# albanie/mcnCrossModalEmotions

Hardware: AMD Instinct MI355X
Metric: distillation-step samples/sec (face+audio pair) (higher is better)
Workload: dtype f32; 1 GPU; BASELINE config 4 shard: frozen resnet50 teacher fwd + VGGVox student fwd/bwd/SGD; per_gpu_batch=32, global_batch=32, face=224x224x3, teacher_batch=32, spectrogram=512x300x1, parallelism=dp1, weights=random-init (seeded), parameter_server=rccl-capi, streams=teacher one batch ahead on its own stream + wgrad side stream

## Files before the change

### mcncrossmodalemotions_amd/csrc/context.cpp

```cpp
#include <cstdlib>
#include <map>
#include <string>
#include <vector>

#include "xm_common.h"

namespace xm {
bool path_on(Path p) {
  static const char *const kEnv[kPathCount] = {"XM_NO_HYBRID",      "XM_NO_HALO",        "XM_NO_SKINNY",     "XM_NO_SKINNY4",
                                               "XM_NO_STEM",        "XM_NO_STEM_WGRAD",  "XM_NO_DMA",        "XM_NO_FUSED_STATS",
                                               "XM_DGRAD_MERGE",    "XM_NO_FAST_TRANSPOSE", "XM_NO_POOL_LDS", "XM_NO_POOL_PATCH",
                                               "XM_NO_POOL_POOLED", "XM_NO_W8", "XM_NO_WGRAD_PATCH", "XM_NO_WGRAD_PATCH_S2", "XM_NO_DGRAD_S2", "XM_NO_STEM3"};
  static bool on[kPathCount];
  static bool read = false;
  if (!read) {
    for (int i = 0; i < kPathCount; ++i) on[i] = getenv(kEnv[i]) == nullptr;
    read = true;
  }
  return on[p];
}

long long env_int(const char *name, long long dflt) {
  const char *e = getenv(name);
  return (e && *e) ? atoll(e) : dflt;
}
double env_double(const char *name, double dflt) {
  const char *e = getenv(name);
  return (e && *e) ? atof(e) : dflt;
}

static char g_err[512] = "";
char *err_buf() { return g_err; }

int fail(int code, const char *fmt, ...) {
  va_list ap;
  va_start(ap, fmt);
  vsnprintf(g_err, sizeof g_err, fmt, ap);
  va_end(ap);
  return code;
}

struct WsBuf {
  void *ptr = nullptr;
  size_t cap = 0;
};
static std::map<hipStream_t, WsBuf> g_ws;
static unsigned long long g_ws_generation = 0;

int ws_get(size_t bytes, void **ptr, hipStream_t stream) {
  WsBuf &w = g_ws[stream];
  if (bytes > w.cap) {
    size_t want = bytes + bytes / 4 + (1u << 20);
    static const bool verbose = getenv("XM_WS_VERBOSE") != nullptr;
    if (verbose) fprintf(stderr, "[xm ws] stream %p grow %zu -> %zu\n", (void *)stream, w.cap, want);
    ++g_ws_generation;
    if (w.ptr) {
      hipError_t e = hipDeviceSynchronize();
      if (e != hipSuccess) return fail(XM_EHIP, "hipDeviceSynchronize -> %s", hipGetErrorString(e));
      (void)hipFree(w.ptr);
      w.ptr = nullptr;
      w.cap = 0;
    }
    hipError_t e = hipMalloc(&w.ptr, want);
    if (e != hipSuccess) {
      w.ptr = nullptr;
      return fail(XM_ENOMEM, "workspace hipMalloc(%zu) -> %s", want, hipGetErrorString(e));
    }
    w.cap = want;
  }
  *ptr = w.ptr;
  return XM_OK;
}

static std::map<std::string, void *> g_tables;

const void *cached_device_table(const void *host, size_t bytes) {
  std::string key((const char *)host, bytes);
  auto it = g_tables.find(key);
  if (it != g_tables.end()) return it->second;
  void *d = nullptr;
  static const bool verbose = getenv("XM_WS_VERBOSE") != nullptr;
  if (verbose) fprintf(stderr, "[xm ws] new device table %zu bytes (#%zu)\n", bytes, g_tables.size());
  if (hipMalloc(&d, bytes) != hipSuccess) return nullptr;
  if (hipMemcpy(d, host, bytes, hipMemcpyHostToDevice) != hipSuccess) {
    (void)hipFree(d);
    return nullptr;
  }
  g_tables.emplace(std::move(key), d);
  return d;
}

}

extern "C" {

int xm_version(void) { return 106; }
const char *xm_last_error(void) { return xm::err_buf(); }

int xm_workspace_reserve(size_t bytes) {
  void *p;
  return xm::ws_get(bytes, &p, nullptr);
}
int xm_workspace_reserve_stream(size_t bytes, void *stream) {
  void *p;
  return xm::ws_get(bytes, &p, (hipStream_t)stream);
}
unsigned long long xm_workspace_generation(void) { return xm::g_ws_generation; }

int xm_device_alloc(void **ptr, size_t bytes) {
  if (!ptr) return xm::fail(XM_EINVAL, "device_alloc: NULL output");
  *ptr = nullptr;
  if (bytes == 0) return XM_OK;
  hipError_t e = hipMalloc(ptr, bytes);
  if (e != hipSuccess) return xm::fail(XM_ENOMEM, "hipMalloc(%zu) -> %s", bytes, hipGetErrorString(e));
  return XM_OK;
}
int xm_device_free(void *ptr) {
  if (!ptr) return XM_OK;
  hipError_t e = hipFree(ptr);
  if (e != hipSuccess) return xm::fail(XM_EHIP, "hipFree -> %s", hipGetErrorString(e));
  return XM_OK;
}
int xm_device_upload(void *dst_device, const void *src_host, size_t bytes) {
  if (bytes == 0) return XM_OK;
// ... 28 lines not shown
```

### mcncrossmodalemotions_amd/csrc/conv.hip

```cpp
#include <dlfcn.h>

#include <algorithm>
#include <climits>
#include <cstdlib>
#include <map>
#include <string>
#include <vector>

#include "conv_kernels.h"
#include "stem_pool_kernels.h"

namespace xm {


__global__ void pad_filter_kernel(const float *__restrict__ f, float *__restrict__ o, int M, int R,
                                  int Rp) {
  size_t i = blockIdx.x * (size_t)blockDim.x + threadIdx.x;
  if (i >= (size_t)M * Rp) return;
  int r = (int)(i % Rp);
  size_t m = i / Rp;
  o[i] = r < R ? f[m * R + r] : 0.f;
}

struct PrepDiv {
// ... 337 lines not shown
  ProfScope(int key, double flops, hipStream_t s, double bytes = 0) : on(g_prof_on), st(s) {
    if (!on) return;
    r.key = key;
    r.flops = flops;
    r.bytes = bytes;
    r.start = prof_event();
    r.stop = prof_event();
    (void)hipEventRecord(r.start, st);
  }
  ~ProfScope() {
    if (!on) return;
    (void)hipEventRecord(r.stop, st);
    g_prof.push_back(r);
  }
};


static const int kCfgOcc[kNumBaseCfg] = {2, 2, 2, 3, 4, 3, 4, 2};

static int hybrid_plan(const ConvGemmArgs &a, int ci, int *full_out) {
  const bool off = !path_on(kPathHybrid);
  *full_out = 0;
  if (off || is_dma_cfg(ci) || g_force_splits > 0) return 1;
  if (a.statPart && (!a.vecStore || a.relu || a.resid)) return 1;
  const int tiles = a.nbm * a.nbn, slots = 256 * kCfgOcc[ci];
  if (tiles <= slots || a.nkt < 16) return 1;
  int full = tiles / slots * slots;
  full -= full % a.nbm;
  const int rem = tiles - full;
  if (rem <= 0 || rem * 5 > slots * 4) return 1;
  const int S = std::min(std::min(slots / rem, a.nkt / 8), 16);
  if (S < 2) return 1;
  *full_out = full;
  return S;
}

static size_t gemm_slab_floats(const ConvGemmArgs &a, int ci, int *splits_out) {
  const Cfg &c = kCfgs[ci];
  int nbm = (a.M + c.bm() - 1) / c.bm(), nbn = (a.NP + c.bn() - 1) / c.bn();
  int splits = pick_splits(nbm * nbn, a.Rp / kBK);
  *splits_out = splits;
  size_t need = splits > 1 ? (size_t)splits * a.M * ((a.NP + 3) & ~3) : 0;
  if (splits == 1 && !is_dma_cfg(ci)) {
    ConvGemmArgs t = a;
    t.nbm = nbm, t.nbn = nbn, t.nkt = a.Rp / kBK;
    t.statPart = nullptr;
    int full;
    const int S = hybrid_plan(t, ci, &full);
    if (S > 1) need = std::max(need, (size_t)S * a.M * ((size_t)(nbm * nbn - full) / nbm * c.bn() + 4));
  }
  return need;
}

static int launch_gemm(ConvGemmArgs &a, int mode, int ci, int splits, float *slab, hipStream_t st) {
  if (is_dma_cfg(ci) && !a.dmaOk) ci = base_cfg(ci);
  if (ci == kCfgW8 && !path_on(kPathW8)) ci = 0;
  const Cfg &c = kCfgs[ci];
  a.nbm = (a.M + c.bm() - 1) / c.bm();
  a.nbn = (a.NP + c.bn() - 1) / c.bn();
  a.nkt = a.Rp / kBK;
  a.tilesPerSplit = (a.nkt + splits - 1) / splits;
  splits = (a.nkt + a.tilesPerSplit - 1) / a.tilesPerSplit;
  a.NPs = (a.NP + 3) & ~3;
  a.slab = splits > 1 ? slab : nullptr;
  a.dbgCycles = g_dbg_cycles;
  a.hyS = 1, a.hyFull = 0, a.hyTps = 0, a.hyP0 = 0;
  dim3 grid(a.nbm * a.nbn, splits);
  int hyS = 1;
  if (splits == 1 && slab) {
    int full;
    hyS = hybrid_plan(a, ci, &full);
    if (hyS > 1) {
      a.hyFull = full;
      a.hyTps = (a.nkt + hyS - 1) / hyS;
      hyS = (a.nkt + a.hyTps - 1) / a.hyTps;
      a.hyS = hyS;
      a.hyP0 = full / a.nbm * c.bn();
      a.NPs = (a.NP - a.hyP0 + 3) & ~3;
      a.slab = slab;
      grid = dim3(full + (a.nbm * a.nbn - full) * hyS, 1);
    }
  }
  {
    const double abytes = (double)a.xBytes + 4.0 * a.M * a.Rtrue + 4.0 * a.M * (double)a.NP * (a.resid ? 2 : 1);
    ProfScope ps(0 * 100 + ci * 2 + mode, a.algoFlops > 0 ? a.algoFlops : 2.0 * a.M * (double)a.NP * a.Rtrue, st,
                 abytes);
    if (is_dma_cfg(ci)) {
      static const int per_cu_tab[] = XM_DMA_PERCU;
      const int slots = std::max(8, 256 * per_cu_tab[ci - kNumBaseCfg] / std::max(1, splits));
      const int ntl = a.nbm * a.nbn;
      const int g = ntl <= slots ? ntl : slots - slots % 8;
      launch_gemm_dma(ci, a, dim3(std::max(1, g), splits), st);
    } else if (mode)
      launch_gemm_cfg<1>(ci, a, grid, st);
    else
      launch_gemm_cfg<0>(ci, a, grid, st);
  }
  XM_LAUNCH_CHECK();
  if (splits > 1 || hyS > 1) {
    const int z = splits > 1 ? splits : hyS;
    const int np = a.NP - a.hyP0;
    const bool vec = a.vecStore && (np & 3) == 0 && (a.hyP0 & 3) == 0 && (a.NPs & 3) == 0 && ((uintptr_t)a.slab & 15) == 0;
    const size_t n = (size_t)a.M * (vec ? np / 4 : np);
    if (hyS > 1 && a.statPart) {
      const int cols = np / 4, chunks = (cols + 255) / 256, statBase = a.hyFull / a.nbm;
      if (!vec) return fail(XM_EINVAL, "vl_nnconv: hybrid schedule with statistics needs vector stores");
      hipLaunchKernelGGL(conv_splitk_epilogue_stats_kernel, dim3(chunks, a.M), dim3(256), 0, st, a, z, cols, statBase);
      a.statNcg = statBase + chunks;
    } else if (vec)
      hipLaunchKernelGGL(conv_splitk_epilogue_kernel<true>, dim3((unsigned)((n + 255) / 256)), dim3(256), 0, st,
                         a, z, make_fastdiv((uint32_t)(np / 4)));
    else
      hipLaunchKernelGGL(conv_splitk_epilogue_kernel<false>, dim3((unsigned)((n + 255) / 256)), dim3(256), 0, st,
                         a, z, make_fastdiv((uint32_t)np));
    XM_LAUNCH_CHECK();
  }
  return XM_OK;
}

static void launch_gemm_multi_cfg(int ci, const ConvGemmMulti &m, dim3 grid, hipStream_t st) {
  dim3 block(cfg_threads(ci));
  switch (ci) {
    case 7: hipLaunchKernelGGL((conv_gemm_multi_kernel<1, 2, 4, 2>), grid, block, 0, st, m); break;
    case 0: hipLaunchKernelGGL((conv_gemm_multi_kernel<2, 2, 2, 2>), grid, block, 0, st, m); break;
    case 1: hipLaunchKernelGGL((conv_gemm_multi_kernel<2, 2, 1, 4>), grid, block, 0, st, m); break;
    case 2: hipLaunchKernelGGL((conv_gemm_multi_kernel<3, 1, 1, 4>), grid, block, 0, st, m); break;
    case 3: hipLaunchKernelGGL((conv_gemm_multi_kernel<1, 2, 2, 2>), grid, block, 0, st, m); break;
    case 4: hipLaunchKernelGGL((conv_gemm_multi_kernel<1, 1, 2, 2>), grid, block, 0, st, m); break;
    case 5: hipLaunchKernelGGL((conv_gemm_multi_kernel<1, 1, 4, 1>), grid, block, 0, st, m); break;
    default: hipLaunchKernelGGL((conv_gemm_multi_kernel<1, 1, 1, 4>), grid, block, 0, st, m); break;
  }
}

static int launch_gemm_multi(const std::vector<ConvGemmArgs> &args, int ci, hipStream_t st) {
  ci = base_cfg(ci);
  if (ci == kCfgW8 && !path_on(kPathW8)) ci = 0;
  const Cfg &c = kCfgs[ci];
  ConvGemmMulti m{};
  int maxTiles = 0;
  double flops = 0, abytes = args.empty() ? 0.0 : (double)args[0].xBytes;
  for (size_t i = 0; i < args.size(); ++i) {
    ConvGemmArgs a = args[i];
    a.nbm = (a.M + c.bm() - 1) / c.bm();
    a.nbn = (a.NP + c.bn() - 1) / c.bn();
    a.nkt = a.Rp / kBK;
    a.tilesPerSplit = a.nkt;
    a.NPs = (a.NP + 3) & ~3;
    a.slab = nullptr;
    maxTiles = std::max(maxTiles, a.nbm * a.nbn);
    flops += a.algoFlops > 0 ? a.algoFlops : 2.0 * a.M * (double)a.NP * a.Rtrue;
    abytes += 4.0 * a.M * a.Rtrue + 4.0 * a.M * (double)a.NP * (a.resid ? 2 : 1);
    m.c[i] = a;
  }
  {
    ProfScope ps(2 * 100 + ci * 2, flops, st, abytes);
    launch_gemm_multi_cfg(ci, m, dim3(maxTiles, 1, (unsigned)args.size()), st);
// ... 35 lines not shown
    const long long p1 = std::min<long long>(p0 + BN - 1, a.NP - 1);
    const long long c0 = (p0 / pij) * a.hpWP + (p0 % pij) / a.PI, c1 = (p1 / pij) * a.hpWP + (p1 % pij) / a.PI;
    worst = std::max(worst, (int)(c1 - c0) + a.nV);
  }
  return worst * a.hpHP;
}
static int halo_setup_padded(ConvGemmArgs &a, int nSamples) {
  int need = halo_setup(a, nSamples);
  if (need <= 512 || a.vecStore || a.slab) return need;
  const int piv = (a.PI + 31) / 32 * 32;
  if (piv == a.PI || (piv - a.PI) * 25 > piv || (long long)piv * a.PJ * nSamples >= (1LL << 31)) return need;
  ConvGemmArgs b = a;
  b.piReal = a.PI;
  b.PI = piv;
  b.NP = piv * a.PJ * nSamples;
  b.divPI = make_fastdiv((uint32_t)piv);
  b.divPIJ = make_fastdiv((uint32_t)(piv * a.PJ));
  const int need2 = halo_setup(b, nSamples);
  if (need2 > 0 && need2 <= 512) {
    a = b;
    return need2;
  }
  return need;
}

static bool halo_var_ok(const ConvGemmArgs &a, int need, int v) {
  if (need <= 0 || need > kHaloVars[v].ps) return false;
  if (v == 2 && need <= 512) return false;
  if (kHaloVars[v].bm == 96 && (a.M % 96 != 0)) return false;
  return true;
}

static int halo_splits(const ConvGemmArgs &a, int v) {
  const int bm = kHaloVars[v].bm;
  const int tiles = ((a.M + bm - 1) / bm) * ((a.NP + 127) / 128), nst = a.Rtrue / (kHaloCB * a.nU * a.nV);
  if (tiles >= 384 || nst < 8) return 1;
  return std::max(1, std::min(std::min(512 / tiles, nst / 4), 16));
}
static size_t halo_slab_floats(const ConvGemmArgs &a) {
  int sp = 1;
  for (int v = 0; v < 3; ++v) sp = std::max(sp, halo_splits(a, v));
  return sp > 1 ? (size_t)sp * a.M * ((a.NP + 3) & ~3) : 0;
}

static void halo_prepare(ConvGemmArgs &a, int v) {
  const int bm = kHaloVars[v].bm;
  a.nbm = (a.M + bm - 1) / bm;
  a.nbn = (a.NP + 127) / 128;
  a.nkt = a.Rtrue / (kHaloCB * a.nU * a.nV);
  a.tilesPerSplit = a.nkt;
  a.NPs = (a.NP + 3) & ~3;
  a.slab = nullptr;
  a.dbgCycles = nullptr;
}

static int forced_halo_variant(const bool *hok) {
  if (g_force_halo >= 1 && g_force_halo <= 3 && hok[g_force_halo]) return g_force_halo;
  return hok[2] ? 2 : (hok[1] ? 1 : 3);
}

static int launch_halo(ConvGemmArgs a, int v, float *slab, hipStream_t st) {
  halo_prepare(a, v);
  int splits = slab ? halo_splits(a, v) : 1;
  a.tilesPerSplit = (a.nkt + splits - 1) / splits;
  splits = (a.nkt + a.tilesPerSplit - 1) / a.tilesPerSplit;
  a.slab = splits > 1 ? slab : nullptr;
  if (a.slab) a.statPart = nullptr;
  {
    const double abytes = (double)a.xBytes + 4.0 * a.M * a.Rtrue + 4.0 * a.M * (double)a.NP * (a.resid ? 2 : 1);
    ProfScope ps(3 * 100 + v, a.algoFlops > 0 ? a.algoFlops : 2.0 * a.M * (double)a.NP * a.Rtrue, st, abytes);
    const dim3 grid(a.nbm * a.nbn, splits), block(256);
    if (v == 0) hipLaunchKernelGGL((conv_halo_kernel<2, 2, 2, 2, 512>), grid, block, 0, st, a);
    else if (v == 1) hipLaunchKernelGGL((conv_halo_kernel<3, 1, 1, 4, 512>), grid, block, 0, st, a);
    else hipLaunchKernelGGL((conv_halo_kernel<3, 1, 1, 4, 1024>), grid, block, 0, st, a);
  }
  XM_LAUNCH_CHECK();
  if (splits > 1) {
    const bool vec = a.vecStore && (a.NP & 3) == 0 && ((uintptr_t)a.slab & 15) == 0;
    const size_t n = (size_t)a.M * (vec ? a.NP / 4 : a.NP);
    if (vec)
      hipLaunchKernelGGL(conv_splitk_epilogue_kernel<true>, dim3((unsigned)((n + 255) / 256)), dim3(256), 0, st,
                         a, splits, make_fastdiv((uint32_t)(a.NP / 4)));
    else
      hipLaunchKernelGGL(conv_splitk_epilogue_kernel<false>, dim3((unsigned)((n + 255) / 256)), dim3(256), 0, st,
                         a, splits, make_fastdiv((uint32_t)a.NP));
    XM_LAUNCH_CHECK();
  }
  return XM_OK;
}

static int launch_halo_multi(const std::vector<ConvGemmArgs> &args, int v, hipStream_t st) {
  ConvGemmMulti m{};
  int maxTiles = 0;
  double flops = 0, abytes = args.empty() ? 0.0 : (double)args[0].xBytes;
  for (size_t i = 0; i < args.size(); ++i) {
    ConvGemmArgs a = args[i];
    halo_prepare(a, v);
    maxTiles = std::max(maxTiles, a.nbm * a.nbn);
    flops += a.algoFlops > 0 ? a.algoFlops : 2.0 * a.M * (double)a.NP * a.Rtrue;
    abytes += 4.0 * a.M * a.Rtrue + 4.0 * a.M * (double)a.NP * (a.resid ? 2 : 1);
    m.c[i] = a;
  }
  {
    ProfScope ps(4 * 100 + v, flops, st, abytes);
    const dim3 grid(maxTiles, 1, (unsigned)args.size()), block(256);
    if (v == 0) hipLaunchKernelGGL((conv_halo_multi_kernel<2, 2, 2, 2, 512>), grid, block, 0, st, m);
    else if (v == 1) hipLaunchKernelGGL((conv_halo_multi_kernel<3, 1, 1, 4, 512>), grid, block, 0, st, m);
    else hipLaunchKernelGGL((conv_halo_multi_kernel<3, 1, 1, 4, 1024>), grid, block, 0, st, m);
  }
  XM_LAUNCH_CHECK();
  return XM_OK;
}

static int choose_cfg(long long M, long long NP, int nkt) {
  return g_force_cfg >= 0 ? g_force_cfg : pick_cfg(M, NP, nkt);
}

struct TuneKey {
  int kind, M, NP, Rp, mode, a, b, c, d;
  bool operator<(const TuneKey &o) const { return memcmp(this, &o, sizeof(TuneKey)) < 0; }
};
static std::map<TuneKey, int> g_tuned;

constexpr int XM_TUNE_REV = 7;
static bool g_tune_loaded = false;
static int g_tune_new = 0;

static std::string tune_default_path() {
  if (const char *e = getenv("XM_TUNE_FILE")) return e;
  Dl_info info;
  if (dladdr((const void *)&tune_default_path, &info) && info.dli_fname) {
    std::string p(info.dli_fname);
// ... 1356 lines not shown
  a.gsx = g.sx;
  a.gh0 = -g.pt;
  a.gw0 = -g.pl;
  a.LimH = g.H;
  a.LimW = g.W;
  a.xSampleStride = g.H * g.W;
}

static int stem_pool_grid(int nunits, int occ) { return std::min(256 * occ, (nunits + 7) / 8 * 8); }
static size_t stem_gram_need(const Geo &g) {
  return WsCarver::need((size_t)stem_pool_grid(stem_pool_units(g), 3) * 64 * 64, 4);
}

static int launch_stem_gram(WsCarver &ws, const float *x, const Geo &g, double *gram, hipStream_t st) {
  StemPoolArgs a{};
  stem_pool_args(a, x, g);
  const int nunits = stem_pool_units(g), grid = stem_pool_grid(nunits, 3);
  a.part = ws.take<float>((size_t)grid * 64 * 64);
  static bool attr_done = false;
  if (!attr_done) {
    XM_HIP(hipFuncSetAttribute((const void *)stem_gram_kernel<2>, hipFuncAttributeMaxDynamicSharedMemorySize, kSpGramSmem));
    XM_HIP(hipFuncSetAttribute((const void *)stem_gram_kernel<1>, hipFuncAttributeMaxDynamicSharedMemorySize, kSpGramSmem));
    attr_done = true;
  }
  {
    ProfScope ps(13 * 100, 2.0 * (g.R + 1) * (g.R + 1) * (double)g.Ho * g.Wo * g.N, st, 4.0 * g.H * g.W * g.N);
    if (g.sy == 2) hipLaunchKernelGGL(stem_gram_kernel<2>, dim3(grid), dim3(256), kSpGramSmem, st, a, nunits);
    else hipLaunchKernelGGL(stem_gram_kernel<1>, dim3(grid), dim3(256), kSpGramSmem, st, a, nunits);
  }
  XM_LAUNCH_CHECK();
  hipLaunchKernelGGL(stem_gram_reduce_kernel, dim3(64), dim3(1024), 0, st, a.part, gram, grid);
  XM_LAUNCH_CHECK();
  return XM_OK;
}

}

using namespace xm;

extern "C" {

int xm_debug_set(const char *key, int value) {
  auto tri = [](int &g, int v) { int old = g; g = v < 0 ? -1 : (v ? 1 : 0); return old; };
  const std::string k = key ? key : "";
  if (k == "conv_cfg") { int old = g_force_cfg; g_force_cfg = (value >= 0 && value < kNumCfg) ? value : -1; return old; }
  if (k == "conv_splits") { int old = g_force_splits; g_force_splits = value > 0 ? value : 0; return old; }
  if (k == "conv_halo") { int old = g_force_halo; g_force_halo = value < 0 ? -1 : std::min(value, 3); return old; }
  if (k == "conv_stem") return tri(g_force_stem, value);
  if (k == "conv_stem3") return tri(g_force_stem3, value);
  if (k == "wgrad_patch") return tri(g_force_wgrad_patch, value);
  if (k == "wgrad_patch_s2") return tri(g_force_wgrad_patch_s2, value);
  if (k == "dgrad_s2") return tri(g_force_dgrad_s2, value);
  if (k == "comm_single") return comm_force_single(value);
  return INT_MIN;
}
int xm_debug_get(const char *key) {
  const std::string k = key ? key : "";
  if (k == "num_conv_cfgs") return kNumCfg;
  if (k == "conv_cfg") return g_force_cfg;
  if (k == "conv_splits") return g_force_splits;
  if (k == "conv_halo") return g_force_halo;
  if (k == "conv_stem") return g_force_stem;
  if (k == "conv_stem3") return g_force_stem3;
  if (k == "wgrad_patch") return g_force_wgrad_patch;
  if (k == "wgrad_patch_s2") return g_force_wgrad_patch_s2;
  if (k == "dgrad_s2") return g_force_dgrad_s2;
  return INT_MIN;
}

int xm_set_exec_hint(unsigned flags) {
  if (flags & ~(unsigned)XM_EXEC_SINGLE_STREAM) return fail(XM_EINVAL, "xm_set_exec_hint: unknown flag bits 0x%x", flags);
  g_exec_hint = flags;
  return XM_OK;
}
unsigned xm_get_exec_hint(void) { return g_exec_hint; }


int xm_tune_load(const char *path) {
  g_tune_loaded = true;
  return tune_load_file(path && path[0] ? path : tune_default_path().c_str());
}
int xm_tune_save(const char *path) {
  tune_load_once();
  std::string p = path && path[0] ? std::string(path) : tune_default_path();
  std::string tmp = p + ".tmp";
  FILE *fp = fopen(tmp.c_str(), "w");
  if (!fp) return fail(XM_EINVAL, "xm_tune_save: cannot write %s", tmp.c_str());
  fprintf(fp, "xmodal-tune 1 rev=%d cfgs=%d\n", XM_TUNE_REV, kNumCfg);
  for (auto &kv : g_tuned) {
    const TuneKey &k = kv.first;
    fprintf(fp, "%d %d %d %d %d %d %d %d %d %d\n", k.kind, k.M, k.NP, k.Rp, k.mode, k.a, k.b, k.c, k.d, kv.second);
  }
  fclose(fp);
  if (rename(tmp.c_str(), p.c_str()) != 0) return fail(XM_EINVAL, "xm_tune_save: rename to %s failed", p.c_str());
  g_tune_new = 0;
  return XM_OK;
}
int xm_tune_entries(int *total, int *unsaved) {
  tune_load_once();
  if (total) *total = (int)g_tuned.size();
  if (unsaved) *unsaved = g_tune_new;
  return XM_OK;
}
#ifdef XM_DEBUG_CYCLES
int xm_debug_conv_cycles(int on, unsigned long long *out, int nblocks) {
  const size_t bytes = 4096 * 4 * sizeof(unsigned long long);
  if (on && !g_dbg_cycles) {
    if (hipMalloc((void **)&g_dbg_cycles, bytes) != hipSuccess) return XM_ENOMEM;
    (void)hipMemset(g_dbg_cycles, 0, bytes);
  }
  if (out && g_dbg_cycles)
    (void)hipMemcpy(out, g_dbg_cycles, (size_t)std::min(nblocks, 4096) * 32, hipMemcpyDeviceToHost);
  if (!on && g_dbg_cycles) {
    (void)hipFree(g_dbg_cycles);
    g_dbg_cycles = nullptr;
  }
  return XM_OK;
}
#endif
// ... 420 lines not shown
```

### mcncrossmodalemotions_amd/csrc/conv_kernels.h

```cpp
#pragma once
#include <type_traits>

#include "xm_common.h"

namespace xm {

typedef float f32x16 __attribute__((ext_vector_type(16)));
typedef float f32x4 __attribute__((ext_vector_type(4)));

struct ConvGemmArgs {
  const float *A;
  const float *X;
  float *Y;
  float *slab;
  const int2 *taps;
  const float *bias, *scale, *shift, *resid;
  const float *gate;
  int gateStride;
  int relu;
  unsigned xBytes;
  unsigned aBytes;
  unsigned tapStride;
  int dmaOk;
  int lda, M, Rp, Rtrue;
  int PI, PJ, NP, NPs;
  FastDiv divPIJ, divPI;
  int gsy, gsx, gh0, gw0;
  int LimH, LimW, xSampleStride;
  int nU, nV, du0, dus, dv0, dvs;
  int osy, osx, oh0, ow0, OH;
  int oChanStride, oSampleStride;
  FastDiv divMU;
  int oUStride;
  int vecStore;
  int nbm, nbn;
  int tilesPerSplit, nkt;
  int hyFull, hyS, hyTps, hyP0;
  float *statPart;
  int statNcg;
  int hpHP, hpWP, hpRmin, hpCmin, hpN;
  int piReal;
  int hpSh[9];
  FastDiv hpDivHP, hpDivWP;
  double algoFlops;
  unsigned long long *dbgCycles;
};

__device__ __forceinline__ int xcd_remap(int bid, int nblk) {
  const int nx = 8;
  int q = nblk / nx, r = nblk % nx;
  int xcd = bid % nx, idx = bid / nx;
  int start = xcd < r ? xcd * (q + 1) : r * (q + 1) + (xcd - r) * q;
  return start + idx;
}

constexpr int kBK = 16;
constexpr int kNG = 4;

__device__ __forceinline__ float buf_load(__amdgpu_buffer_rsrc_t r, unsigned byte_off) {
  return __builtin_bit_cast(float, __builtin_amdgcn_raw_buffer_load_b32(r, (int)byte_off, 0, 0));
}
template <int AV>
__device__ __forceinline__ auto buf_load_v(__amdgpu_buffer_rsrc_t r, unsigned byte_off) {
  if constexpr (AV == 4) {
    typedef unsigned u4 __attribute__((ext_vector_type(4)));
    typedef float f4 __attribute__((ext_vector_type(4)));
    u4 v = __builtin_amdgcn_raw_buffer_load_b128(r, (int)byte_off, 0, 0);
    return __builtin_bit_cast(f4, v);
  } else {
    typedef unsigned u2 __attribute__((ext_vector_type(2)));
    typedef float f2 __attribute__((ext_vector_type(2)));
    u2 v = __builtin_amdgcn_raw_buffer_load_b64(r, (int)byte_off, 0, 0);
    return __builtin_bit_cast(f2, v);
  }
}

__device__ __forceinline__ float dpp_quad(float x, const int ctrl_is_xor1) {
  int xi = __builtin_bit_cast(int, x);
  int r = ctrl_is_xor1 ? __builtin_amdgcn_mov_dpp(xi, 0xB1, 0xF, 0xF, true)
                       : __builtin_amdgcn_mov_dpp(xi, 0x4E, 0xF, 0xF, true);
  return __builtin_bit_cast(float, r);
}
__device__ __forceinline__ void quad_transpose4(float (&v)[4], int iq) {
  const bool b0 = iq & 1, b1 = iq & 2;
  float s0 = b0 ? v[0] : v[1], s1 = b0 ? v[2] : v[3];
  s0 = dpp_quad(s0, 1);
  s1 = dpp_quad(s1, 1);
  if (b0) { v[0] = s0; v[2] = s1; } else { v[1] = s0; v[3] = s1; }
  float t0 = b1 ? v[0] : v[2], t1 = b1 ? v[1] : v[3];
  t0 = dpp_quad(t0, 0);
// ... 9 lines not shown
  xi = __builtin_bit_cast(int, x);
  x += __builtin_bit_cast(float, __builtin_amdgcn_ds_swizzle(xi, 0x401F));
  return x;
}

#define XM_SGB_VALU 0x002
#define XM_SGB_MFMA 0x008
#define XM_SGB_VMEM_RD 0x020
#define XM_SGB_DS_RD 0x100
#define XM_SGB_DS_WR 0x200

#define XM_MFMA_E(E, AF, BF)                                                   \
  _Pragma("unroll") for (int i = 0; i < TM; ++i)                               \
    _Pragma("unroll") for (int j = 0; j < TN; ++j) {                           \
      if (TM * TN == 1 && ((E) & 1))                                           \
        accx = __builtin_amdgcn_mfma_f32_32x32x2f32(AF[i][E], BF[j][E], accx, 0, 0, 0); \
      else                                                                     \
        acc[i][j] = __builtin_amdgcn_mfma_f32_32x32x2f32(AF[i][E], BF[j][E], acc[i][j], 0, 0, 0); \
    }
#define XM_MFMA_CHUNK(AF, BF)                                                  \
  XM_MFMA_E(0, AF, BF)                                                         \
  XM_MFMA_E(1, AF, BF)                                                         \
  XM_MFMA_E(2, AF, BF)                                                         \
  XM_MFMA_E(3, AF, BF)
#define XM_READ_FRAGS(CUR, S, AF, BF)                                          \
  _Pragma("unroll") for (int i = 0; i < TM; ++i)                               \
    AF[i] = *reinterpret_cast<const f32x4 *>(sAr + ((CUR) * kNG + 2 * (S)) * PLA + i * 128); \
  _Pragma("unroll") for (int j = 0; j < TN; ++j)                               \
    BF[j] = *reinterpret_cast<const f32x4 *>(sBr + ((CUR) * kNG + 2 * (S)) * PLB + j * 128);

#define XM_INTERLEAVE(NVALU)                                                   \
  __builtin_amdgcn_sched_group_barrier(XM_SGB_DS_RD, TM + TN, 0);              \
  _Pragma("unroll") for (int q_ = 0; q_ < 4 * TM * TN; ++q_) {                 \
    __builtin_amdgcn_sched_group_barrier(XM_SGB_MFMA, 1, 0);                   \
    __builtin_amdgcn_sched_group_barrier(XM_SGB_VALU, NVALU, 0);              \
    __builtin_amdgcn_sched_group_barrier(XM_SGB_VMEM_RD, 1, 0);                \
  }

template <bool ASMST>
__device__ __forceinline__ void xm_st16(float *p, f32x4 v) {
  if constexpr (ASMST)
    asm volatile("global_store_dwordx4 %0, %1, off\n\ts_nop 1" ::"v"(p), "v"(v) : "memory");
  else
    *reinterpret_cast<f32x4 *>(p) = v;
}
template <bool ASMST>
__device__ __forceinline__ void xm_st4(float *p, float v) {
  if constexpr (ASMST)
    asm volatile("global_store_dword %0, %1, off" ::"v"(p), "v"(v) : "memory");
  else
    *p = v;
}

template <int TM, int TN, int WGM, int WGN, bool ASMST = false>
__device__ __forceinline__ void conv_gemm_epilogue(const ConvGemmArgs &a, f32x16 (&acc)[TM][TN], int bm, int bn,
                                                   int split, int wm, int wn, int half, int l31,
                                                   float *sred = nullptr ,
                                                   bool toSlab = true ) {
  constexpr int BM = 32 * TM * WGM, BN = 32 * TN * WGN;
  if (a.slab && toSlab) {
    float *out = a.slab + (size_t)split * a.M * a.NPs - a.hyP0;
#pragma unroll
    for (int j = 0; j < TN; ++j) {
      int p = bn * BN + (wn * TN + j) * 32 + l31;
      if (p >= a.NP) continue;
#pragma unroll
      for (int i = 0; i < TM; ++i)
#pragma unroll
        for (int r = 0; r < 16; ++r) {
          int m = bm * BM + (wm * TM + i) * 32 + (r & 3) + 8 * (r >> 2) + 4 * half;
          if (m < a.M) xm_st4<ASMST>(out + (size_t)m * a.NPs + p, acc[i][j][r]);
        }
    }
    return;
  }
  const int wbase = __builtin_amdgcn_readfirstlane(bm * BM + wm * TM * 32);
  int obase[TN], gbase[TN];
  bool pok[TN];
#pragma unroll
  for (int j = 0; j < TN; ++j) {
    int p = bn * BN + (wn * TN + j) * 32 + l31;
    pok[j] = p < a.NP;
    uint32_t pc = pok[j] ? p : a.NP - 1;
    uint32_t n = xm_div(pc, a.divPIJ);
    gbase[j] = (int)n * a.gateStride;
    uint32_t q = pc - n * a.divPIJ.d;
    uint32_t jj = xm_div(q, a.divPI);
    uint32_t ii = q - jj * a.divPI.d;
    obase[j] = (a.oh0 + (int)ii * a.osy) + a.OH * (a.ow0 + (int)jj * a.osx) + (int)n * a.oSampleStride;
    if (a.piReal) pok[j] = pok[j] && (int)ii < a.piReal;
  }
  if (a.vecStore) {
    const int iq = l31 & 3;
    float rmul[TM][4], radd[TM][4];
    {
      int rowc[TM][4];
      float bi_[TM][4];
#pragma unroll
      for (int i = 0; i < TM; ++i)
#pragma unroll
        for (int g4 = 0; g4 < 4; ++g4) {
          rowc[i][g4] = min(wbase + i * 32 + 8 * g4 + 4 * half + iq, a.M - 1);
          rmul[i][g4] = 1.f;
          radd[i][g4] = 0.f;
          bi_[i][g4] = 0.f;
        }
      if (a.scale) {
#pragma unroll
        for (int i = 0; i < TM; ++i)
#pragma unroll
          for (int g4 = 0; g4 < 4; ++g4) {
            rmul[i][g4] = a.scale[rowc[i][g4]];
            radd[i][g4] = a.shift[rowc[i][g4]];
          }
      }
      if (a.bias) {
#pragma unroll
        for (int i = 0; i < TM; ++i)
#pragma unroll
          for (int g4 = 0; g4 < 4; ++g4) bi_[i][g4] = a.bias[rowc[i][g4]];
#pragma unroll
        for (int i = 0; i < TM; ++i)
#pragma unroll
          for (int g4 = 0; g4 < 4; ++g4) radd[i][g4] += bi_[i][g4] * rmul[i][g4];
      }
    }
// ... 1556 lines not shown
        for (int e = 0; e < 4; ++e) {
          const int s = 4 * c + e;
          const float *px = sW + (s < w ? b0 : b1) + SY * s;
          float bv[2];
#pragma unroll
          for (int jt = 0; jt < 2; ++jt) bv[jt] = px[tapoff[jt]];
          if (ONES) bv[ONES ? ONES - 1 : 0] = onesLane ? 1.f : bv[ONES ? ONES - 1 : 0];
#pragma unroll
          for (int jt = 0; jt < 2; ++jt) acc[i][jt] = __builtin_amdgcn_mfma_f32_32x32x2f32(af[e], bv[jt], acc[i][jt], 0, 0, 0);
        }
        if (c == 1) {
          __builtin_amdgcn_sched_barrier(0);
          decode_write(xc, prt, 0);
          pooled_issue(prt, 1);
          __builtin_amdgcn_sched_barrier(0);
        }
      }
      __builtin_amdgcn_sched_barrier(0);
      decode_write(xc, prt, 1);
      if (i == 2) write_patch();
#pragma unroll
      for (int kk = 0; kk < 4; ++kk) xc[kk] = xn[kk];
    }
    cur = nxt;
  }
  float *const sD = smem;
  for (int wq = 0; wq < 4; ++wq) {
    __syncthreads();
    if (wave == wq) {
#pragma unroll
      for (int i = 0; i < TM; ++i)
#pragma unroll
        for (int jt = 0; jt < 2; ++jt)
#pragma unroll
          for (int r = 0; r < 16; ++r) {
            float *d = sD + (32 * i + (r & 3) + 8 * (r >> 2) + 4 * half) * 64 + 32 * jt + l31;
            *d = wq ? *d + acc[i][jt][r] : acc[i][jt][r];
          }
    }
  }
  __syncthreads();
  float *out = a.part + (size_t)blockIdx.x * (96 * 64);
  for (int i = t; i < 96 * 64 / 4; i += 256) reinterpret_cast<f32x4 *>(out)[i] = reinterpret_cast<const f32x4 *>(sD)[i];
}

template <bool VEC>
__global__ void __launch_bounds__(256)
conv_splitk_epilogue_kernel(const ConvGemmArgs a, int splits, FastDiv divCols) {
  const uint32_t idx = blockIdx.x * 256u + threadIdx.x;
  const uint32_t cols = divCols.d;
  if (idx >= (uint32_t)a.M * cols) return;
  const int m = (int)xm_div(idx, divCols);
  const int pr = (int)(idx - (uint32_t)m * cols) * (VEC ? 4 : 1);
  const int p = pr + a.hyP0;
  uint32_t n = xm_div((uint32_t)p, a.divPIJ);
  uint32_t q = (uint32_t)p - n * a.divPIJ.d;
  uint32_t jj = xm_div(q, a.divPI);
  uint32_t ii = q - jj * a.divPI.d;
  uint32_t mc = xm_div((uint32_t)m, a.divMU);
  int off = (a.oh0 + (int)ii * a.osy) + a.OH * (a.ow0 + (int)jj * a.osx) + (int)n * a.oSampleStride +
            (int)mc * a.oChanStride + (m - (int)mc * (int)a.divMU.d) * a.oUStride;
  if (VEC) {
    f32x4 v = {0.f, 0.f, 0.f, 0.f};
    for (int z = 0; z < splits; ++z) v += *reinterpret_cast<const f32x4 *>(a.slab + ((size_t)z * a.M + m) * a.NPs + pr);
    if (a.bias) v += a.bias[m];
    if (a.scale) v = v * a.scale[m] + a.shift[m];
    if (a.gate) v *= a.gate[m + (int)n * a.gateStride];
    if (a.resid) v += *reinterpret_cast<const f32x4 *>(a.resid + off);
    if (a.relu) {
      v.x = fmaxf(v.x, 0.f);
      v.y = fmaxf(v.y, 0.f);
      v.z = fmaxf(v.z, 0.f);
      v.w = fmaxf(v.w, 0.f);
    }
    *reinterpret_cast<f32x4 *>(a.Y + off) = v;
  } else {
    float v = 0.f;
    for (int z = 0; z < splits; ++z) v += a.slab[((size_t)z * a.M + m) * a.NPs + pr];
    if (a.bias) v += a.bias[m];
    if (a.scale) v = v * a.scale[m] + a.shift[m];
    if (a.gate) v *= a.gate[m + (int)n * a.gateStride];
    if (a.resid) v += a.resid[off];
    if (a.relu) v = fmaxf(v, 0.f);
    a.Y[off] = v;
  }
}

__global__ void __launch_bounds__(256)
conv_splitk_epilogue_stats_kernel(const ConvGemmArgs a, int splits, int cols, int statBase) {
  __shared__ float red[2][4];
  const int m = blockIdx.y, c = blockIdx.x * 256 + threadIdx.x;
  float s1 = 0.f, s2 = 0.f;
  if (c < cols) {
    const int pr = c * 4, p = pr + a.hyP0;
    const uint32_t n = xm_div((uint32_t)p, a.divPIJ);
    const uint32_t q = (uint32_t)p - n * a.divPIJ.d;
    const uint32_t jj = xm_div(q, a.divPI);
    const uint32_t ii = q - jj * a.divPI.d;
    const uint32_t mc = xm_div((uint32_t)m, a.divMU);
    const int off = (a.oh0 + (int)ii * a.osy) + a.OH * (a.ow0 + (int)jj * a.osx) + (int)n * a.oSampleStride +
                    (int)mc * a.oChanStride + (m - (int)mc * (int)a.divMU.d) * a.oUStride;
    f32x4 v = {0.f, 0.f, 0.f, 0.f};
    for (int z = 0; z < splits; ++z) v += *reinterpret_cast<const f32x4 *>(a.slab + ((size_t)z * a.M + m) * a.NPs + pr);
    float rmul = 1.f, radd = 0.f;
    if (a.scale) rmul = a.scale[m], radd = a.shift[m];
    if (a.bias) radd += a.bias[m] * rmul;
    v = v * rmul + radd;
    if (a.gate) v *= a.gate[m + (int)n * a.gateStride];
    s1 = (v.x + v.y) + (v.z + v.w);
    s2 = (v.x * v.x + v.y * v.y) + (v.z * v.z + v.w * v.w);
    *reinterpret_cast<f32x4 *>(a.Y + off) = v;
  }
  s1 = xm_wave_sum(s1);
  s2 = xm_wave_sum(s2);
  const int wv = threadIdx.x >> 6;
  if ((threadIdx.x & 63) == 0) red[0][wv] = s1, red[1][wv] = s2;
  __syncthreads();
  if (threadIdx.x == 0)
    *reinterpret_cast<float2 *>(a.statPart + ((size_t)(statBase + blockIdx.x) * a.M + m) * 2) =
        make_float2((red[0][0] + red[0][1]) + (red[0][2] + red[0][3]), (red[1][0] + red[1][1]) + (red[1][2] + red[1][3]));
}

struct WgradArgs {
  const float *dY;
  const float *X;
  float *out;
  const int4 *taps;
  unsigned xBytes, dyBytes;
  int M, R, Rn, ldo;
  int Ho, Wo, NP;
  FastDiv divHW, divHo;
  int sy, sx, pt, pl_;
  int H, W, xSampleStride;
  int dyChanStride, dySampleStride;
  int nbm, nbn, tilesPerSplit, nkt;
  size_t splitStride;
};
// ... 721 lines not shown
```

### mcncrossmodalemotions_amd/csrc/xm_common.h

```cpp
#pragma once
#include <hip/hip_runtime.h>

#include <cstdarg>
#include <cstdint>
#include <cstdio>
#include <cstring>

#include "../../include/xmodal.h"

namespace xm {

char *err_buf();
int fail(int code, const char *fmt, ...);

#define XM_HIP(expr)                                                                  \
  do {                                                                                \
    hipError_t e__ = (expr);                                                          \
    if (e__ != hipSuccess)                                                            \
      return xm::fail(XM_EHIP, "%s -> %s (%s:%d)", #expr, hipGetErrorString(e__), __FILE__, __LINE__); \
  } while (0)

#define XM_LAUNCH_CHECK()                                                             \
  do {                                                                                \
    hipError_t e__ = hipGetLastError();                                               \
    if (e__ != hipSuccess)                                                            \
      return xm::fail(XM_EHIP, "kernel launch -> %s (%s:%d)", hipGetErrorString(e__), __FILE__, __LINE__); \
  } while (0)

int ws_get(size_t bytes, void **ptr, hipStream_t stream);
struct WsCarver {
  char *base = nullptr;
  size_t off = 0, cap = 0;
  int init(size_t bytes, hipStream_t stream) {
    void *p = nullptr;
    int rc = ws_get(bytes, &p, stream);
    base = (char *)p;
    cap = bytes;
    off = 0;
    return rc;
  }
  template <class T>
  T *take(size_t count) {
    size_t b = (count * sizeof(T) + 255) & ~size_t(255);
    T *p = (T *)(base + off);
    off += b;
    return p;
  }
  static size_t need(size_t count, size_t elt) { return (count * elt + 255) & ~size_t(255); }
};

enum Path {
  kPathHybrid,
  kPathHalo,
  kPathSkinny,
  kPathSkinny4,
  kPathStem,
  kPathStemWgrad,
  kPathDma,
  kPathFusedStats,
  kPathDgradMerge,
  kPathFastTranspose,
  kPathPoolLds,
  kPathPoolPatch,
  kPathPoolPooled,
  kPathW8,
  kPathWgradPatch,
  kPathWgradPatchS2,
  kPathDgradS2,
  kPathStem3,
  kPathCount
};
bool path_on(Path p);
long long env_int(const char *name, long long dflt);
double env_double(const char *name, double dflt);

int comm_force_single(int on);

const void *cached_device_table(const void *host, size_t bytes);

int bn_batch_moments(const float *x, int H, int W, int C, int N, float eps, float *moments_out, hipStream_t st);

size_t bnpool_sums_need(int C, int N);
// ... 53 lines not shown
```

Before: 4093 pairs/s.

## Fold split-K reduction into GEMM via last-block counters and vectorize slab stores

Adds an in-kernel split-K fold for conv GEMMs. Each split writes its partial tile to the slab and bumps a per-tile atomic counter, and the last-arriving workgroup sums all splits and applies the fused epilogue (bias, scale, gate, residual, ReLU). This removes the separate split-K epilogue launch and one pass over the slab. The fold only turns on through a debug knob or when the slab size fits under XM_SPLITK_FOLD_KB, which defaults to 0, so by default only the new vectorized (quad-transposed 16-byte) slab stores take effect. The change also adds device counters per stream and extra fences and atomics when folding is enabled.

```diff
diff --git a/mcncrossmodalemotions_amd/csrc/context.cpp b/mcncrossmodalemotions_amd/csrc/context.cpp
--- a/mcncrossmodalemotions_amd/csrc/context.cpp
+++ b/mcncrossmodalemotions_amd/csrc/context.cpp
@@ -70,6 +70,23 @@
   }
   *ptr = w.ptr;
   return XM_OK;
+}
+
+static std::map<hipStream_t, int *> g_splitk_cnt;
+
+int *splitk_counters(hipStream_t stream) {
+  auto it = g_splitk_cnt.find(stream);
+  if (it != g_splitk_cnt.end()) return it->second;
+  hipStreamCaptureStatus cs = hipStreamCaptureStatusNone;
+  if (hipStreamIsCapturing(stream, &cs) != hipSuccess || cs != hipStreamCaptureStatusNone) return nullptr;
+  int *d = nullptr;
+  if (hipMalloc(&d, kSplitkCounters * sizeof(int)) != hipSuccess) return nullptr;
+  if (hipMemsetAsync(d, 0, kSplitkCounters * sizeof(int), stream) != hipSuccess) {
+    (void)hipFree(d);
+    return nullptr;
+  }
+  g_splitk_cnt.emplace(stream, d);
+  return d;
 }
 
 static std::map<std::string, void *> g_tables;
diff --git a/mcncrossmodalemotions_amd/csrc/conv.hip b/mcncrossmodalemotions_amd/csrc/conv.hip
--- a/mcncrossmodalemotions_amd/csrc/conv.hip
+++ b/mcncrossmodalemotions_amd/csrc/conv.hip
@@ -413,6 +413,16 @@
   return need;
 }
 
+static int g_splitk_fold = -1;
+static int g_splitk_combines = 0;
+static const long long kFoldKB = env_int("XM_SPLITK_FOLD_KB", 0);
+
+static int *fold_counters(const ConvGemmArgs &a, int S, int tiles, int bm, int bn, hipStream_t st) {
+  if (g_splitk_fold == 0 || S < 2 || tiles > kSplitkCounters) return nullptr;
+  if (g_splitk_fold != 2 && (long long)S * bm * bn * 4 > kFoldKB * 1024) return nullptr;
+  return splitk_counters(st);
+}
+
 static int launch_gemm(ConvGemmArgs &a, int mode, int ci, int splits, float *slab, hipStream_t st) {
   if (is_dma_cfg(ci) && !a.dmaOk) ci = base_cfg(ci);
   if (ci == kCfgW8 && !path_on(kPathW8)) ci = 0;
@@ -442,6 +452,15 @@
       grid = dim3(full + (a.nbm * a.nbn - full) * hyS, 1);
     }
   }
+  a.foldS = splits > 1 ? splits : hyS;
+  a.slabVec = 0;
+  a.foldCnt = nullptr;
+  if (a.foldS > 1) {
+    const int np = a.NP - a.hyP0;
+    a.slabVec = a.vecStore && (np & 3) == 0 && (a.hyP0 & 3) == 0 && (a.NPs & 3) == 0 && ((uintptr_t)a.slab & 15) == 0;
+    if (!is_dma_cfg(ci) && ci != kCfgW8 && !(hyS > 1 && a.statPart))
+      a.foldCnt = fold_counters(a, a.foldS, a.nbm * a.nbn - a.hyFull, c.bm(), c.bn(), st);
+  }
   {
     const double abytes = (double)a.xBytes + 4.0 * a.M * a.Rtrue + 4.0 * a.M * (double)a.NP * (a.resid ? 2 : 1);
     ProfScope ps(0 * 100 + ci * 2 + mode, a.algoFlops > 0 ? a.algoFlops : 2.0 * a.M * (double)a.NP * a.Rtrue, st,
@@ -458,11 +477,12 @@
       launch_gemm_cfg<0>(ci, a, grid, st);
   }
   XM_LAUNCH_CHECK();
-  if (splits > 1 || hyS > 1) {
-    const int z = splits > 1 ? splits : hyS;
+  if ((splits > 1 || hyS > 1) && !a.foldCnt) {
+    const int z = a.foldS;
     const int np = a.NP - a.hyP0;
-    const bool vec = a.vecStore && (np & 3) == 0 && (a.hyP0 & 3) == 0 && (a.NPs & 3) == 0 && ((uintptr_t)a.slab & 15) == 0;
+    const bool vec = a.slabVec;
     const size_t n = (size_t)a.M * (vec ? np / 4 : np);
+    ++g_splitk_combines;
     if (hyS > 1 && a.statPart) {
       const int cols = np / 4, chunks = (cols + 255) / 256, statBase = a.hyFull / a.nbm;
       if (!vec) return fail(XM_EINVAL, "vl_nnconv: hybrid schedule with statistics needs vector stores");
@@ -604,6 +624,8 @@
   a.NPs = (a.NP + 3) & ~3;
   a.slab = nullptr;
   a.dbgCycles = nullptr;
+  a.hyS = 1, a.hyFull = 0, a.hyTps = 0, a.hyP0 = 0;
+  a.slabVec = 0, a.foldS = 1, a.foldCnt = nullptr;
 }
 
 static int forced_halo_variant(const bool *hok) {
@@ -617,7 +639,12 @@
   a.tilesPerSplit = (a.nkt + splits - 1) / splits;
   splits = (a.nkt + a.tilesPerSplit - 1) / a.tilesPerSplit;
   a.slab = splits > 1 ? slab : nullptr;
-  if (a.slab) a.statPart = nullptr;
+  if (a.slab) {
+    a.statPart = nullptr;
+    a.foldS = splits;
+    a.slabVec = a.vecStore && (a.NP & 3) == 0 && ((uintptr_t)a.slab & 15) == 0;
+    a.foldCnt = fold_counters(a, splits, a.nbm * a.nbn, kHaloVars[v].bm, 128, st);
+  }
   {
     const double abytes = (double)a.xBytes + 4.0 * a.M * a.Rtrue + 4.0 * a.M * (double)a.NP * (a.resid ? 2 : 1);
     ProfScope ps(3 * 100 + v, a.algoFlops > 0 ? a.algoFlops : 2.0 * a.M * (double)a.NP * a.Rtrue, st, abytes);
@@ -627,9 +654,10 @@
     else hipLaunchKernelGGL((conv_halo_kernel<3, 1, 1, 4, 1024>), grid, block, 0, st, a);
   }
   XM_LAUNCH_CHECK();
-  if (splits > 1) {
-    const bool vec = a.vecStore && (a.NP & 3) == 0 && ((uintptr_t)a.slab & 15) == 0;
+  if (splits > 1 && !a.foldCnt) {
+    const bool vec = a.slabVec;
     const size_t n = (size_t)a.M * (vec ? a.NP / 4 : a.NP);
+    ++g_splitk_combines;
     if (vec)
       hipLaunchKernelGGL(conv_splitk_epilogue_kernel<true>, dim3((unsigned)((n + 255) / 256)), dim3(256), 0, st,
                          a, splits, make_fastdiv((uint32_t)(a.NP / 4)));
@@ -2092,6 +2120,7 @@
   if (k == "wgrad_patch_s2") return tri(g_force_wgrad_patch_s2, value);
   if (k == "dgrad_s2") return tri(g_force_dgrad_s2, value);
   if (k == "comm_single") return comm_force_single(value);
+  if (k == "splitk_fold") { int old = g_splitk_fold; g_splitk_fold = value < 0 ? -1 : std::min(value, 2); return old; }
   return INT_MIN;
 }
 int xm_debug_get(const char *key) {
@@ -2105,6 +2134,8 @@
   if (k == "wgrad_patch") return g_force_wgrad_patch;
   if (k == "wgrad_patch_s2") return g_force_wgrad_patch_s2;
   if (k == "dgrad_s2") return g_force_dgrad_s2;
+  if (k == "splitk_fold") return g_splitk_fold;
+  if (k == "splitk_combines") return g_splitk_combines;
   return INT_MIN;
 }
 
diff --git a/mcncrossmodalemotions_amd/csrc/conv_kernels.h b/mcncrossmodalemotions_amd/csrc/conv_kernels.h
--- a/mcncrossmodalemotions_amd/csrc/conv_kernels.h
+++ b/mcncrossmodalemotions_amd/csrc/conv_kernels.h
@@ -36,6 +36,8 @@
   int nbm, nbn;
   int tilesPerSplit, nkt;
   int hyFull, hyS, hyTps, hyP0;
+  int slabVec, foldS;
+  int *foldCnt;
   float *statPart;
   int statNcg;
   int hpHP, hpWP, hpRmin, hpCmin, hpN;
@@ -151,6 +153,142 @@
     *p = v;
 }
 
+__device__ __forceinline__ int splitk_out_offset(const ConvGemmArgs &a, int m, int pr, uint32_t &n) {
+  const int p = pr + a.hyP0;
+  n = xm_div((uint32_t)p, a.divPIJ);
+  uint32_t q = (uint32_t)p - n * a.divPIJ.d;
+  uint32_t jj = xm_div(q, a.divPI);
+  uint32_t ii = q - jj * a.divPI.d;
+  uint32_t mc = xm_div((uint32_t)m, a.divMU);
+  return (a.oh0 + (int)ii * a.osy) + a.OH * (a.ow0 + (int)jj * a.osx) + (int)n * a.oSampleStride +
+         (int)mc * a.oChanStride + (m - (int)mc * (int)a.divMU.d) * a.oUStride;
+}
+__device__ __forceinline__ void splitk_finish(const ConvGemmArgs &a, int m, int pr, f32x4 v) {
+  uint32_t n;
+  const int off = splitk_out_offset(a, m, pr, n);
+  if (a.bias) v += a.bias[m];
+  if (a.scale) v = v * a.scale[m] + a.shift[m];
+  if (a.gate) v *= a.gate[m + (int)n * a.gateStride];
+  if (a.resid) v += *reinterpret_cast<const f32x4 *>(a.resid + off);
+  if (a.relu) {
+    v.x = fmaxf(v.x, 0.f);
+    v.y = fmaxf(v.y, 0.f);
+    v.z = fmaxf(v.z, 0.f);
+    v.w = fmaxf(v.w, 0.f);
+  }
+  *reinterpret_cast<f32x4 *>(a.Y + off) = v;
+}
+__device__ __forceinline__ void splitk_finish(const ConvGemmArgs &a, int m, int pr, float v) {
+  uint32_t n;
+  const int off = splitk_out_offset(a, m, pr, n);
+  if (a.bias) v += a.bias[m];
+  if (a.scale) v = v * a.scale[m] + a.shift[m];
+  if (a.gate) v *= a.gate[m + (int)n * a.gateStride];
+  if (a.resid) v += a.resid[off];
+  if (a.relu) v = fmaxf(v, 0.f);
+  a.Y[off] = v;
+}
+
+template <int BM, int BN, int NT>
+__device__ __forceinline__ void splitk_fold(const ConvGemmArgs &a, int bm, int bn, float *sflag) {
+  asm volatile("s_waitcnt vmcnt(0)" ::: "memory");
+  __syncthreads();
+  const int ci = bm + bn * a.nbm - a.hyFull;
+  int *lflag = reinterpret_cast<int *>(sflag);
+  if (threadIdx.x == 0) {
+    __builtin_amdgcn_fence(__ATOMIC_RELEASE, "agent");
+    asm volatile("s_waitcnt vmcnt(0)" ::: "memory");
+    const int ticket = __hip_atomic_fetch_add(a.foldCnt + ci, 1, __ATOMIC_RELAXED, __HIP_MEMORY_SCOPE_AGENT);
+    const int last = ticket == a.foldS - 1;
+    if (last) {
+      __builtin_amdgcn_fence(__ATOMIC_ACQUIRE, "agent");
+      asm volatile("s_waitcnt vmcnt(0)" ::: "memory");
+      __hip_atomic_store(a.foldCnt + ci, 0, __ATOMIC_RELAXED, __HIP_MEMORY_SCOPE_AGENT);
+    }
+    *lflag = last;
+  }
+  __syncthreads();
+  if (!*lflag) return;
+  const int m0 = bm * BM, p0 = bn * BN, S = a.foldS;
+  const size_t zs = (size_t)a.M * a.NPs;
+  constexpr int ZB = 4;
+  if (a.slabVec) {
+    constexpr int QR = BN / 4, NQ = BM * QR, U = 4;
+    for (int q0 = threadIdx.x; q0 < NQ; q0 += U * NT) {
+      f32x4 v[U];
+      int m[U], pr[U];
+      bool ok[U];
+#pragma unroll
+      for (int u = 0; u < U; ++u) {
+        const int e = q0 + u * NT;
+        m[u] = m0 + e / QR;
+        const int p = p0 + 4 * (e % QR);
+        ok[u] = e < NQ && m[u] < a.M && p < a.NP;
+        pr[u] = p - a.hyP0;
+        v[u] = f32x4{0.f, 0.f, 0.f, 0.f};
+      }
+      const float *src[U];
+#pragma unroll
+      for (int u = 0; u < U; ++u) src[u] = a.slab + (ok[u] ? (size_t)m[u] * a.NPs + pr[u] : 0);
+      int z = 0;
+      for (; z + ZB <= S; z += ZB) {
+        f32x4 t[ZB][U];
+#pragma unroll
+        for (int k = 0; k < ZB; ++k)
+#pragma unroll
+          for (int u = 0; u < U; ++u) t[k][u] = *reinterpret_cast<const f32x4 *>(src[u] + (z + k) * zs);
+#pragma unroll
+        for (int k = 0; k < ZB; ++k)
+#pragma unroll
+          for (int u = 0; u < U; ++u) v[u] += t[k][u];
+      }
+      for (; z < S; ++z)
+#pragma unroll
+        for (int u = 0; u < U; ++u) v[u] += *reinterpret_cast<const f32x4 *>(src[u] + z * zs);
+#pragma unroll
+      for (int u = 0; u < U; ++u)
+        if (ok[u]) splitk_finish(a, m[u], pr[u], v[u]);
+    }
+  } else {
+    constexpr int NE = BM * BN, U = 8;
+    for (int e0 = threadIdx.x; e0 < NE; e0 += U * NT) {
+      float v[U];
+      int m[U], pr[U];
+      bool ok[U];
+#pragma unroll
+      for (int u = 0; u < U; ++u) {
+        const int e = e0 + u * NT;
+        m[u] = m0 + e / BN;
+        const int p = p0 + e % BN;
+        ok[u] = e < NE && m[u] < a.M && p < a.NP;
+        pr[u] = p - a.hyP0;
+        v[u] = 0.f;
+      }
+      const float *src[U];
+#pragma unroll
+      for (int u = 0; u < U; ++u) src[u] = a.slab + (ok[u] ? (size_t)m[u] * a.NPs + pr[u] : 0);
+      int z = 0;
+      for (; z + ZB <= S; z += ZB) {
+        float t[ZB][U];
+#pragma unroll
+        for (int k = 0; k < ZB; ++k)
+#pragma unroll
+          for (int u = 0; u < U; ++u) t[k][u] = src[u][(z + k) * zs];
+#pragma unroll
+        for (int k = 0; k < ZB; ++k)
+#pragma unroll
+          for (int u = 0; u < U; ++u) v[u] += t[k][u];
+      }
+      for (; z < S; ++z)
+#pragma unroll
+        for (int u = 0; u < U; ++u) v[u] += src[u][z * zs];
+#pragma unroll
+      for (int u = 0; u < U; ++u)
+        if (ok[u]) splitk_finish(a, m[u], pr[u], v[u]);
+    }
+  }
+}
+
 template <int TM, int TN, int WGM, int WGN, bool ASMST = false>
 __device__ __forceinline__ void conv_gemm_epilogue(const ConvGemmArgs &a, f32x16 (&acc)[TM][TN], int bm, int bn,
                                                    int split, int wm, int wn, int half, int l31,
@@ -159,18 +297,39 @@
   constexpr int BM = 32 * TM * WGM, BN = 32 * TN * WGN;
   if (a.slab && toSlab) {
     float *out = a.slab + (size_t)split * a.M * a.NPs - a.hyP0;
-#pragma unroll
-    for (int j = 0; j < TN; ++j) {
-      int p = bn * BN + (wn * TN + j) * 32 + l31;
-      if (p >= a.NP) continue;
-#pragma unroll
-      for (int i = 0; i < TM; ++i)
-#pragma unroll
-        for (int r = 0; r < 16; ++r) {
-          int m = bm * BM + (wm * TM + i) * 32 + (r & 3) + 8 * (r >> 2) + 4 * half;
-          if (m < a.M) xm_st4<ASMST>(out + (size_t)m * a.NPs + p, acc[i][j][r]);
-        }
-    }
+    if (WGM * WGN == 4 && a.slabVec) {
+      const int iq = l31 & 3;
+#pragma unroll
+      for (int j = 0; j < TN; ++j) {
+        const int p = bn * BN + (wn * TN + j) * 32 + l31 - iq;
+#pragma unroll
+        for (int i = 0; i < TM; ++i)
+#pragma unroll
+          for (int g4 = 0; g4 < 4; ++g4) {
+            float v[4];
+#pragma unroll
+            for (int k = 0; k < 4; ++k) v[k] = acc[i][j][4 * g4 + k];
+            quad_transpose4(v, iq);
+            const int m = bm * BM + (wm * TM + i) * 32 + 8 * g4 + 4 * half + iq;
+            if (m < a.M && p < a.NP) xm_st16<ASMST>(out + (size_t)m * a.NPs + p, f32x4{v[0], v[1], v[2], v[3]});
+          }
+      }
+    } else {
+#pragma unroll
+      for (int j = 0; j < TN; ++j) {
+        int p = bn * BN + (wn * TN + j) * 32 + l31;
+        if (p >= a.NP) continue;
+#pragma unroll
+        for (int i = 0; i < TM; ++i)
+#pragma unroll
+          for (int r = 0; r < 16; ++r) {
+            int m = bm * BM + (wm * TM + i) * 32 + (r & 3) + 8 * (r >> 2) + 4 * half;
+            if (m < a.M) xm_st4<ASMST>(out + (size_t)m * a.NPs + p, acc[i][j][r]);
+          }
+      }
+    }
+    if constexpr (!ASMST && WGM * WGN == 4)
+      if (a.foldCnt) splitk_fold<BM, BN, 64 * WGM * WGN>(a, bm, bn, sred);
     return;
   }
   const int wbase = __builtin_amdgcn_readfirstlane(bm * BM + wm * TM * 32);
@@ -1833,37 +1992,14 @@
   if (idx >= (uint32_t)a.M * cols) return;
   const int m = (int)xm_div(idx, divCols);
   const int pr = (int)(idx - (uint32_t)m * cols) * (VEC ? 4 : 1);
-  const int p = pr + a.hyP0;
-  uint32_t n = xm_div((uint32_t)p, a.divPIJ);
-  uint32_t q = (uint32_t)p - n * a.divPIJ.d;
-  uint32_t jj = xm_div(q, a.divPI);
-  uint32_t ii = q - jj * a.divPI.d;
-  uint32_t mc = xm_div((uint32_t)m, a.divMU);
-  int off = (a.oh0 + (int)ii * a.osy) + a.OH * (a.ow0 + (int)jj * a.osx) + (int)n * a.oSampleStride +
-            (int)mc * a.oChanStride + (m - (int)mc * (int)a.divMU.d) * a.oUStride;
   if (VEC) {
     f32x4 v = {0.f, 0.f, 0.f, 0.f};
     for (int z = 0; z < splits; ++z) v += *reinterpret_cast<const f32x4 *>(a.slab + ((size_t)z * a.M + m) * a.NPs + pr);
-    if (a.bias) v += a.bias[m];
-    if (a.scale) v = v * a.scale[m] + a.shift[m];
-    if (a.gate) v *= a.gate[m + (int)n * a.gateStride];
-    if (a.resid) v += *reinterpret_cast<const f32x4 *>(a.resid + off);
-    if (a.relu) {
-      v.x = fmaxf(v.x, 0.f);
-      v.y = fmaxf(v.y, 0.f);
-      v.z = fmaxf(v.z, 0.f);
-      v.w = fmaxf(v.w, 0.f);
-    }
-    *reinterpret_cast<f32x4 *>(a.Y + off) = v;
+    splitk_finish(a, m, pr, v);
   } else {
     float v = 0.f;
     for (int z = 0; z < splits; ++z) v += a.slab[((size_t)z * a.M + m) * a.NPs + pr];
-    if (a.bias) v += a.bias[m];
-    if (a.scale) v = v * a.scale[m] + a.shift[m];
-    if (a.gate) v *= a.gate[m + (int)n * a.gateStride];
-    if (a.resid) v += a.resid[off];
-    if (a.relu) v = fmaxf(v, 0.f);
-    a.Y[off] = v;
+    splitk_finish(a, m, pr, v);
   }
 }
 
diff --git a/mcncrossmodalemotions_amd/csrc/xm_common.h b/mcncrossmodalemotions_amd/csrc/xm_common.h
--- a/mcncrossmodalemotions_amd/csrc/xm_common.h
+++ b/mcncrossmodalemotions_amd/csrc/xm_common.h
@@ -28,6 +28,8 @@
   } while (0)
 
 int ws_get(size_t bytes, void **ptr, hipStream_t stream);
+constexpr int kSplitkCounters = 4096;
+int *splitk_counters(hipStream_t stream);
 struct WsCarver {
   char *base = nullptr;
   size_t off = 0, cap = 0;
```

After: 4082 pairs/s (median of 2 runs). Within noise of the previous version (-0.3%).
